# SingleRust/SingleRust

Hardware: AMD Instinct MI355X
Metric: cells/sec end-to-end normalise->HVG->50-PC PCA; SpMM achieved HBM GB/s vs peak (higher is better)
Workload: dtype f32

## Files before the change

### singlerust_amd/csrc/pca_solve.hip

```cpp
#include "pca_internal.hpp"

namespace srx {

#include "spmm.inl"

#include "iterate.inl"

template <typename VT, typename PT>
static int32_t launch_fwd(srx_ctx* ctx, const Tiled& c, const PT* P, const PT* cvec, PT* Y, double* scores = nullptr,
                          int n_pc = 0, int ld = 0) {
    const double out_bytes = scores ? (double)c.n_rows * n_pc * 8.0 : (double)c.n_rows * L * sizeof(PT);
    const double bytes = (double)c.nnz * (4.0 + sizeof(VT)) + (double)((uint64_t)c.nt * c.n_rows + 1) * 8.0 + out_bytes +
                         (double)c.k * L * sizeof(PT);
    const size_t lds = (size_t)KT * L * sizeof(PT);
    constexpr int kRowsPerWg = (kFwdThreads / 16) * FwdCfg<PT>::kRows;
    const uint64_t n_blocks = (c.n_rows + kRowsPerWg - 1) / kRowsPerWg;
    const int per_cu = sizeof(PT) == 4 ? 2 : 1;
    uint64_t grid = (uint64_t)ctx->n_cus * per_cu;
    if (grid > n_blocks) grid = n_blocks;
    if (grid < 1) grid = 1;
    ProfScope ps(ctx, SRX_K_SPMM_FWD, bytes);
    SRX_HIP(ctx, hipFuncSetAttribute((const void*)k_spmm_fwd<VT, PT>, hipFuncAttributeMaxDynamicSharedMemorySize,
                                     (int)lds));
    hipLaunchKernelGGL((k_spmm_fwd<VT, PT>), dim3((unsigned)grid), dim3(kFwdThreads), lds, ctx->stream, c.tptr,
                       (const GramPk<VT>*)c.tpk, c.n_rows, c.nt, c.k, P, cvec, Y, scores, n_pc, ld ? ld : n_pc);
    SRX_HIP(ctx, hipGetLastError());
    return SRX_OK;
}

template <typename PT>
static int fwd_rows_q(int k) {
    const size_t budget = 163840 - 64;
    for (int q = sizeof(PT) == 4 ? 4 : 2; q >= 1; q >>= 1)
        if ((size_t)k * 4 * q * sizeof(PT) <= budget) return q;
    return 0;
}

template <typename VT, typename PT>
static int32_t launch_fwd_rows(srx_ctx* ctx, const RowMajor& r, const PT* P, const PT* cvec, int n_cols, double* scores, PT* Y,
                               int ld) {
    const int Qr = fwd_rows_q<PT>(r.k);
    auto go = [&](auto qtag, auto rtag, auto cltag, int k_lo, int k_hi, int accumulate) -> int32_t {
        constexpr int Q = decltype(qtag)::value;
        constexpr bool RANGE = decltype(rtag)::value;
        constexpr int CL = decltype(cltag)::value;
        constexpr int C = CL * Q;
        const int n_slices = (n_cols + C - 1) / C;
        const int ldp = C;
        const size_t lds = (size_t)(k_hi - k_lo) * ldp * sizeof(PT);
        const uint64_t groups = kFwdRowsThreads / Q;
        uint64_t n_wg = (r.n_rows + groups - 1) / groups;
        uint64_t cap = std::max<uint64_t>(1, (uint64_t)ctx->n_cus * 8 / n_slices);
        if (cap > 8) cap &= ~(uint64_t)7;
        if (n_wg > cap) n_wg = cap;
        if (n_wg < 1) n_wg = 1;
        const double out_bytes = scores ? (double)r.n_rows * n_cols * 8.0 : (double)r.n_rows * L * sizeof(PT);
        ProfScope ps(ctx, SRX_K_SPMM_FWD, (double)r.nnz * sizeof(GramPk<VT>) + (double)(r.n_rows + 1) * 8.0 + out_bytes +
                                              (double)(k_hi - k_lo) * L * sizeof(PT) + (r.perm ? (double)r.n_rows * 4.0 : 0.0));
        SRX_HIP(ctx, hipFuncSetAttribute((const void*)k_spmm_rows<VT, PT, Q, RANGE, CL>, hipFuncAttributeMaxDynamicSharedMemorySize, (int)lds));
        hipLaunchKernelGGL((k_spmm_rows<VT, PT, Q, RANGE, CL>), dim3((unsigned)(n_wg * n_slices)), dim3(kFwdRowsThreads), lds, ctx->stream,
                           r.ptr, (const GramPk<VT>*)r.pk, (const uint32_t*)r.perm, r.n_rows, r.k, P, cvec, n_cols, scores, Y, ld, ldp,
                           k_lo, k_hi, accumulate, 0);
        SRX_HIP(ctx, hipGetLastError());
        return SRX_OK;
    };
    using No = std::false_type;
    using Yes = std::true_type;
    using C4 = std::integral_constant<int, 4>;
    using C5 = std::integral_constant<int, 5>;
    constexpr int Qmax = sizeof(PT) == 4 ? 4 : 2;
    const int wide_slices = (n_cols + 5 * Qmax - 1) / (5 * Qmax), narrow_slices = (n_cols + 4 * Qmax - 1) / (4 * Qmax);
    const bool wide = Qr == Qmax && (size_t)r.k * 5 * Qmax * sizeof(PT) <= (size_t)163840 && wide_slices < narrow_slices &&
                      wide_slices * 5 * Qmax <= L && sizeof(PT) == 8;
    if (wide) return go(std::integral_constant<int, Qmax>{}, No{}, C5{}, 0, r.k, 0);
    if (Qr == 4) {
        if constexpr (sizeof(PT) == 4) return go(std::integral_constant<int, 4>{}, No{}, C4{}, 0, r.k, 0);
        else return SRX_E_ARG;
    }
    if (Qr == 2) return go(std::integral_constant<int, 2>{}, No{}, C4{}, 0, r.k, 0);
    if (Qr == 1) return go(std::integral_constant<int, 1>{}, No{}, C4{}, 0, r.k, 0);
    const int per = (int)((163840 - 64) / (4 * sizeof(PT)));
    for (int k_lo = 0, i = 0; k_lo < r.k; k_lo += per, ++i)
        SRX_TRY(go(std::integral_constant<int, 1>{}, Yes{}, C4{}, k_lo, std::min(r.k, k_lo + per), i > 0 ? 1 : 0));
    return SRX_OK;
}

int32_t build_row_order(srx_ctx* ctx, RowMajor& r) {
    uint32_t* hist;
    SRX_TRY(scratch(ctx, "pca_rm_lenhist", kLenBins * sizeof(uint32_t), (void**)&hist));
    SRX_TRY(scratch(ctx, "pca_rm_perm", (r.n_rows ? r.n_rows : 1) * sizeof(uint32_t), (void**)&r.perm));
    SRX_HIP(ctx, hipMemsetAsync(hist, 0, kLenBins * sizeof(uint32_t), ctx->stream));
    const unsigned g = (unsigned)((r.n_rows + kLenRowsPerWg - 1) / kLenRowsPerWg + (r.n_rows ? 0 : 1));
    hipLaunchKernelGGL(k_len_hist, dim3(g), dim3(256), 0, ctx->stream, r.ptr, r.n_rows, hist);
    hipLaunchKernelGGL(k_len_scan, dim3(1), dim3(kLenBins), 0, ctx->stream, hist);
    hipLaunchKernelGGL(k_len_scatter, dim3(g), dim3(256), 0, ctx->stream, r.ptr, r.n_rows, hist, r.perm);
    SRX_HIP(ctx, hipGetLastError());
    return SRX_OK;
}

template <typename VT, typename YT>
static int32_t launch_t(srx_ctx* ctx, const Tiled& c, const YT* Y, double* T ) {
    uint64_t want = (uint64_t)(2 * ctx->n_cus) / (uint64_t)c.nt;
    if (want < 1) want = 1;
    uint64_t by_rows = (c.n_rows + 255) / 256;
    if (by_rows < 1) by_rows = 1;
    const uint64_t n_rb = want < by_rows ? want : by_rows;
    const uint64_t rpb = (c.n_rows + n_rb - 1) / n_rb > 0 ? (c.n_rows + n_rb - 1) / n_rb : 1;
    double *part, *part_s;
    SRX_TRY(scratch(ctx, "pca_tpart", n_rb * (size_t)c.k * L * sizeof(double), (void**)&part));
    SRX_TRY(scratch(ctx, "pca_tpart_s", n_rb * L * sizeof(double), (void**)&part_s));
    const size_t lds = (size_t)KT * L * sizeof(double);
    const double bytes = (double)c.nnz * (4.0 + sizeof(VT)) + (double)((uint64_t)c.nt * c.n_rows + 1) * 8.0 +
                         (double)c.n_rows * L * sizeof(YT) + (double)c.k * L * 8.0;
    {
        ProfScope ps(ctx, SRX_K_SPMM_T, bytes);
        SRX_HIP(ctx, hipFuncSetAttribute((const void*)k_spmm_t<VT, YT, double>,
                                         hipFuncAttributeMaxDynamicSharedMemorySize, (int)lds));
        hipLaunchKernelGGL((k_spmm_t<VT, YT, double>), dim3((unsigned)(n_rb * c.nt)), dim3(kTThreads), lds, ctx->stream,
                           c.tptr, (const GramPk<VT>*)c.tpk, c.n_rows, c.k, c.nt, rpb, Y, part, part_s);
        uint64_t tot = (uint64_t)c.k * L + L;
        hipLaunchKernelGGL((k_t_reduce<double>), dim3((unsigned)((tot + 255) / 256)), dim3(256), 0, ctx->stream, part,
                           part_s, c.k, n_rb, T);
    }
    SRX_HIP(ctx, hipGetLastError());
    return SRX_OK;
}

static uint64_t mix64(uint64_t x) {
    x += 0x9E3779B97F4A7C15ull;
    x = (x ^ (x >> 30)) * 0xBF58476D1CE4E5B9ull;
    x = (x ^ (x >> 27)) * 0x94D049BB133111EBull;
    return x ^ (x >> 31);
}

struct Work {
    double *W, *Wp, *T, *A1, *A2, *small, *mu, *d, *gpart;
    double *dHG, *dM, *dM2, *dTheta, *dRho, *dColmax, *dSgn, *dDinv, *dXi;
};

static int32_t alloc_work(srx_ctx* ctx, int k, Work& w) {
    const size_t kl = (size_t)k * L;
    SRX_TRY(scratch(ctx, "pca_W", kl * 8, (void**)&w.W));
    SRX_TRY(scratch(ctx, "pca_Wp", kl * 8, (void**)&w.Wp));
    SRX_TRY(scratch(ctx, "pca_T", (kl + L) * 8, (void**)&w.T));
    SRX_TRY(scratch(ctx, "pca_A1", kl * 8, (void**)&w.A1));
    SRX_TRY(scratch(ctx, "pca_A2", kl * 8, (void**)&w.A2));
    SRX_TRY(scratch(ctx, "pca_small", (6 * L * L + 8 * L + 4 * 16 * 16) * 8, (void**)&w.small));
    SRX_TRY(scratch(ctx, "pca_mu", (size_t)k * 8, (void**)&w.mu));
    SRX_TRY(scratch(ctx, "pca_d", (size_t)k * 8, (void**)&w.d));
    SRX_TRY(scratch(ctx, "pca_g2part", (size_t)kGram2Blocks * 2 * L * L * 8, (void**)&w.gpart));
    w.dHG = w.small;
    w.dM = w.small + 2 * L * L;
    w.dM2 = w.small + 3 * L * L;
    w.dTheta = w.small + 4 * L * L;
    w.dRho = w.dTheta + L;
    w.dColmax = w.dRho + L;
    w.dSgn = w.dColmax + L;
    w.dDinv = w.dSgn + L;
    w.dXi = w.small + 6 * L * L + 8 * L;
    return SRX_OK;
}

static int32_t gram2(srx_ctx* ctx, const Work& w, const double* A, const double* B, int k) {
    int nb = (k + 31) / 32;
    if (nb > kGram2Blocks) nb = kGram2Blocks;
    if (nb < 1) nb = 1;
    hipLaunchKernelGGL(k_gram2_part, dim3(nb), dim3(1024), 0, ctx->stream, A, B, k, w.gpart);
    hipLaunchKernelGGL(k_gram2_reduce, dim3((2 * L * L + 255) / 256), dim3(256), 0, ctx->stream, w.gpart, nb, w.dHG);
    SRX_HIP(ctx, hipGetLastError());
    return SRX_OK;
}

template <typename Fn>
static int32_t graphed(srx_ctx* ctx, bool enable, const std::string& key, Fn&& enqueue) {
    if (!enable || ctx->graphs_off) return enqueue();
    auto it = ctx->graphs.find(key);
    if (it == ctx->graphs.end()) {
        if (ctx->graphs.size() >= 32) {
            for (auto& kv : ctx->graphs) (void)hipGraphExecDestroy(kv.second);
            ctx->graphs.clear();
        }
        if (hipStreamBeginCapture(ctx->stream, hipStreamCaptureModeRelaxed) != hipSuccess) {
            (void)hipGetLastError();
            ctx->graphs_off = true;
            return enqueue();
        }
        ctx->capturing = true;
        const int32_t rc = enqueue();
        ctx->capturing = false;
        hipGraph_t g = nullptr;
        const hipError_t e = hipStreamEndCapture(ctx->stream, &g);
        hipGraphExec_t ex = nullptr;
        if (rc == SRX_OK && e == hipSuccess && g && hipGraphInstantiate(&ex, g, nullptr, nullptr, 0) == hipSuccess) {
            (void)hipGraphDestroy(g);
            it = ctx->graphs.emplace(key, ex).first;
        } else {
            if (g) (void)hipGraphDestroy(g);
            (void)hipGetLastError();
            ctx->graphs_off = true;
            return rc != SRX_OK ? rc : enqueue();
        }
    }
    SRX_HIP(ctx, hipGraphLaunch(it->second, ctx->stream));
    return SRX_OK;
}

template <typename Apply>
static int32_t subspace_iterate(srx_ctx* ctx, const Work& w, int k, int l_act, const Resolved& o, Apply&& apply,
                                const void* apply_id, bool graphable, const int* d_status_sel, double& resid, int& iters,
                                bool& converged, bool acc_apply, bool resume = false, bool* bailed_first = nullptr) {
    const size_t kl = (size_t)k * L;
    const bool use_graph = graphable && !getenv("SRX_NO_GRAPH");
    const bool use_cheb = l_act > o.n_pc && !o.robust && !o.direct;
    constexpr int kSlots = srx_ctx::kAsyncSlots, kSlotDoubles = 8;
    if (!ctx->pin_async) {
        SRX_HIP(ctx, hipHostMalloc((void**)&ctx->pin_async, kSlots * kSlotDoubles * sizeof(double), hipHostMallocDefault));
        for (auto& e : ctx->async_ev) SRX_HIP(ctx, hipEventCreateWithFlags(&e, hipEventDisableTiming));
    }
    int* d_status;
    double* d_res;
    constexpr size_t kStatusBytes = 256;
    SRX_TRY(scratch(ctx, "pca_status", kStatusBytes + (size_t)L * L * sizeof(double), (void**)&d_status));
    double* const d_h1 = reinterpret_cast<double*>(reinterpret_cast<char*>(d_status) + kStatusBytes);
    SRX_TRY(scratch(ctx, "pca_res", kSlots * kSlotDoubles * sizeof(double), (void**)&d_res));
    double* d_ritz;
    SRX_TRY(scratch(ctx, "pca_ritzpart", (size_t)kRitzBlocks * 3 * L * sizeof(double), (void**)&d_ritz));
    SRX_HIP(ctx, hipFuncSetAttribute((const void*)k_jacobi_eig2, hipFuncAttributeMaxDynamicSharedMemorySize, (int)sizeof(J2Lds)));
    char key0[320];
    snprintf(key0, sizeof key0, "k%d l%d p%d w%d r%d n%d s%llu t%a|%p %p %p %p %p %p %p %p %p %p", k, l_act, o.power, o.warm,
             (o.robust ? 1 : 0) + (o.direct ? 2 : 0) + (acc_apply ? 4 : 0), o.n_pc,
             (unsigned long long)o.seed, o.tol, apply_id, (void*)w.W, (void*)w.Wp, (void*)w.A1, (void*)w.A2, (void*)w.small,
             (void*)w.gpart, (void*)d_status, (void*)d_status_sel, (void*)w.T);
    const std::string key_base(key0);


    auto gram1 = [&](const double* A, const double* B) -> int32_t {
        int nb = (k + 31) / 32;
        if (nb > kGram1Blocks) nb = kGram1Blocks;
        hipLaunchKernelGGL(k_gram1_part, dim3(nb), dim3(1024), 0, ctx->stream, A, B, k, d_h1);
        SRX_HIP(ctx, hipGetLastError());
        return 1;
    };
    auto orth = [&](const double* src) -> int32_t {
        if (o.robust) {
            SRX_TRY(gram2(ctx, w, src, src, k));
            hipLaunchKernelGGL(k_chol_factor, dim3(1), dim3(1024), 0, ctx->stream, w.dHG + L * L, l_act, w.dM, w.dDinv, d_status, 1);
        } else {
            const int32_t nb = gram1(src, src);
            if (nb < 0) return nb;
            hipLaunchKernelGGL(k_chol_factor_mfma, dim3(1), dim3(1024), 0, ctx->stream, d_h1, l_act, w.dM, w.dDinv, w.dXi, d_status);
        }
        double* const zT = acc_apply ? w.T : nullptr;
        double* const zWp = acc_apply ? w.Wp : nullptr;
        double* const zA1 = acc_apply ? w.A1 : nullptr;
        if (o.robust)
            hipLaunchKernelGGL(k_trsm_rows, dim3((k + 63) / 64), dim3(64), 0, ctx->stream, src, (const double*)w.dM, (const double*)w.dDinv, k, w.W, zWp, zA1, zT);
        else
            hipLaunchKernelGGL(k_trsm_mfma, dim3((k + 16 * kTrsmTiles - 1) / (16 * kTrsmTiles)), dim3(kTrsmTiles * 64), 0, ctx->stream, src,
                               (const double*)w.dM, (const double*)w.dXi, k, w.W, zWp, zA1, zT);
        SRX_HIP(ctx, hipGetLastError());
        if (o.robust) {
            SRX_TRY(gram2(ctx, w, w.W, w.W, k));
            hipLaunchKernelGGL(k_chol_factor, dim3(1), dim3(1024), 0, ctx->stream, w.dHG + L * L, l_act, w.dM, w.dDinv, d_status, 1);
            hipLaunchKernelGGL(k_trsm_rows, dim3((k + 63) / 64), dim3(64), 0, ctx->stream, (const double*)w.W, (const double*)w.dM, (const double*)w.dDinv, k, w.W,
                               (double*)nullptr, (double*)nullptr, (double*)nullptr);
            SRX_HIP(ctx, hipGetLastError());
        }
        return SRX_OK;
    };
    auto apply_n = [&](const double* src, int n, bool after_orth, const double** out) -> int32_t {
        const double* cur = src;
        double* const cand[3] = {w.Wp, w.A1, acc_apply ? w.T : nullptr};
        bool zero[3] = {acc_apply, acc_apply && after_orth, acc_apply};
        for (int t = 0; t < n; ++t) {
            int pick = -1;
            for (int c = 0; c < 3 && pick < 0; ++c)
                if (cand[c] && cand[c] != cur && zero[c]) pick = c;
            for (int c = 0; c < 3 && pick < 0; ++c)
                if (cand[c] && cand[c] != cur) pick = c;
            SRX_TRY(apply(cur, cand[pick], zero[pick]));
            zero[pick] = false;
            cur = cand[pick];
        }
        *out = cur;
        return SRX_OK;
    };
    auto ritz_kernels = [&](int slot, bool loose = false, bool wp_zero = false) -> int32_t {
        SRX_TRY(apply(w.W, w.Wp, wp_zero || acc_apply));
        {
            const int32_t nb = gram1(w.W, w.Wp);
            if (nb < 0) return nb;
            constexpr double loose_tol2 = 1e-6;
            const double exact_tol2 = std::max(1e-30, (o.tol * 1e-4) * (o.tol * 1e-4));
            hipLaunchKernelGGL(k_jacobi_eig2, dim3(1), dim3(kJ2Threads), sizeof(J2Lds), ctx->stream, d_h1, l_act,
                               w.dM2, w.dTheta, d_status, loose ? loose_tol2 : exact_tol2,
                               o.direct ? l_act : std::min(l_act, o.n_pc + 4));
            hipLaunchKernelGGL(k_ritz_post, dim3(kRitzBlocks), dim3(256), 0, ctx->stream, (const double*)w.W, w.Wp,
                               (const double*)w.dM2, (const double*)w.dTheta, k, w.A1, w.A2, d_ritz, acc_apply ? 1 : 0);
            hipLaunchKernelGGL(k_resid_final, dim3(1), dim3(1024), 0, ctx->stream, (const double*)d_ritz, kRitzBlocks,
                               (const double*)w.dTheta, o.n_pc, l_act, d_status, d_status_sel, w.dRho, w.dColmax,
                               d_res + kSlotDoubles * slot);
        }
        SRX_HIP(ctx, hipGetLastError());
        return SRX_OK;
    };
    auto ritz_readback = [&](int slot) -> int32_t {
        SRX_HIP(ctx, hipMemcpyAsync(ctx->pin_async + kSlotDoubles * slot, d_res + kSlotDoubles * slot,
                                    kSlotDoubles * sizeof(double), hipMemcpyDeviceToHost, ctx->stream));
        SRX_HIP(ctx, hipEventRecord(ctx->async_ev[slot], ctx->stream));
        return SRX_OK;
    };
    auto advance = [&]() -> int32_t {
        const double* res;
        SRX_TRY(apply_n(w.A1, o.power - 1, false, &res));
        return orth(res);
    };
    double spread = 1.0;
    auto collect = [&](int slot, double& r, double& ratio) -> int32_t {
        SRX_HIP(ctx, hipEventSynchronize(ctx->async_ev[slot]));
        r = ctx->pin_async[kSlotDoubles * slot];
        const int st = (int)ctx->pin_async[kSlotDoubles * slot + 1];
        ratio = ctx->pin_async[kSlotDoubles * slot + 2];
        spread = ctx->pin_async[kSlotDoubles * slot + 4];
        if ((int)ctx->pin_async[kSlotDoubles * slot + 3] & 1)
            return fail(ctx, SRX_E_NAN, "NaN gene variance: called `Option::unwrap()` on a `None` value (partial_cmp)");
        if (st & kStatChol) return fail(ctx, SRX_E_NOCONV, "pca: block lost rank (Cholesky pivot <= 0)");
        if (st & kStatEig) return fail(ctx, SRX_E_NOCONV, "pca: l x l eigen-solver did not converge");
        if (r != r) return fail(ctx, SRX_E_NOCONV, "pca: NaN in the Ritz residual");
        return SRX_OK;
    };
    auto plain_sweep = [&]() -> int32_t {
        const double* res;
        SRX_TRY(apply_n(w.W, o.power, true, &res));
        return orth(res);
    };

    auto seg_start = [&]() -> int32_t {
        if (o.direct) {
            SRX_HIP(ctx, hipMemsetAsync(d_status, 0, kStatusBytes + (size_t)L * L * sizeof(double), ctx->stream));
            hipLaunchKernelGGL(k_identity_block, dim3((unsigned)((kl + 255) / 256)), dim3(256), 0, ctx->stream, k, w.W);
            SRX_HIP(ctx, hipGetLastError());
            if (acc_apply) SRX_HIP(ctx, hipMemsetAsync(w.Wp, 0, kl * 8, ctx->stream));
            return ritz_kernels(0, false);
        }
        const bool start_orth = o.robust || o.warm < 1;
        hipLaunchKernelGGL(k_init_block, dim3((unsigned)((kl + 255) / 256)), dim3(256), 0, ctx->stream, o.seed, k, l_act,
                           start_orth ? w.Wp : w.W, acc_apply && !start_orth ? w.Wp : (double*)nullptr,
                           acc_apply ? w.A1 : (double*)nullptr, acc_apply ? w.T : (double*)nullptr, reinterpret_cast<uint32_t*>(d_status),
                           (int)((kStatusBytes + (size_t)L * L * sizeof(double)) / 4));
        if (start_orth) {
            SRX_TRY(orth(w.Wp));
            SRX_TRY(orth(w.W));
        }
        for (int sweep = 0; sweep < o.warm; ++sweep) SRX_TRY(plain_sweep());
        return ritz_kernels(0, true);
    };
    const unsigned cheb_grid = (unsigned)((kl + 255) / 256);
    auto cheb_spec = [&]() -> int32_t {
        hipLaunchKernelGGL(k_cheb_first, dim3(cheb_grid), dim3(256), 0, ctx->stream, w.A1, (const double*)w.A2,
                           (const double*)w.dTheta, l_act, kl);
        SRX_HIP(ctx, hipGetLastError());
        return apply(w.A1, w.Wp, acc_apply);
    };
    auto cheb_filter = [&](int d) -> int32_t {
        double *cur = w.A1, *prev = w.A2;
        for (int j = 1; j < d; ++j) {
            if (j > 1) SRX_TRY(apply(cur, w.Wp, true));
            hipLaunchKernelGGL(k_cheb_step, dim3(cheb_grid), dim3(256), 0, ctx->stream, w.Wp,
                               (const double*)cur, prev, (const double*)w.dTheta, l_act, kl);
            double* t = cur;
            cur = prev;
            prev = t;
        }
        hipLaunchKernelGGL(k_cheb_scale, dim3(cheb_grid), dim3(256), 0, ctx->stream, cur, (const double*)w.dTheta, l_act, d, kl);
        SRX_HIP(ctx, hipGetLastError());
        return orth(cur);
    };
    auto cheb_rest = [&](int d, int d2, int slot) -> int32_t {
        SRX_TRY(cheb_filter(d));
        if (d2 > 0) {
            SRX_TRY(apply(w.W, w.Wp, acc_apply));
            hipLaunchKernelGGL(k_cheb_first2, dim3(cheb_grid), dim3(256), 0, ctx->stream, w.Wp, (const double*)w.W, w.A1, w.A2,
                               (const double*)w.dTheta, l_act, kl);
            SRX_HIP(ctx, hipGetLastError());
            SRX_TRY(apply(w.A1, w.Wp, true));
            SRX_TRY(cheb_filter(d2));
        }
        return ritz_kernels(slot, false, true);
    };
    auto seg_next = [&](bool with_advance, int m, int slot) -> int32_t {
        if (with_advance) SRX_TRY(advance());
        for (int sI = 1; sI < m; ++sI) SRX_TRY(plain_sweep());
        return ritz_kernels(slot);
    };

    resid = INFINITY;
    converged = false;
    iters = 0;
    int n_ritz = 0, slot = 0;
    int q_applied = o.warm * o.power + 1;
    double r_last = INFINITY, rate_meas = 0.0;
    int sweeps_since = 0;
    if (bailed_first) *bailed_first = false;
    if (resume) {
        hipLaunchKernelGGL(k_resid_final, dim3(1), dim3(1024), 0, ctx->stream, (const double*)d_ritz, kRitzBlocks,
                           (const double*)w.dTheta, o.n_pc, l_act, d_status, d_status_sel, w.dRho, w.dColmax, d_res + kSlotDoubles * slot);
        SRX_HIP(ctx, hipGetLastError());
    } else {
        SRX_TRY(graphed(ctx, use_graph, key_base + "|start", seg_start));
    }
    SRX_TRY(ritz_readback(slot));
    for (;;) {
        ++iters;
        ++n_ritz;
        const bool first = n_ritz == 1;
        const bool cheb = use_cheb;
        if (cheb && first) {
            if (!resume) SRX_TRY(graphed(ctx, use_graph, key_base + "|cheb0", cheb_spec));
        } else if (first && !o.direct) SRX_TRY(graphed(ctx, use_graph, key_base + "|adv", advance));
        double r, ratio;
        SRX_TRY(collect(slot, r, ratio));
        resid = r;
        if (getenv("SRX_PCA_TRACE")) {
            fprintf(stderr, "[srx pca] sweep %d (ritz step %d): residual %.3e, theta_l/theta_npc %.3e, %d Jacobi sweeps\n", iters + o.warm,
                    n_ritz, r, ratio, (int)ctx->pin_async[kSlotDoubles * slot + 5]);
            int st[64];
            if (d2h(ctx, st, d_status, sizeof st) == SRX_OK) {
                fprintf(stderr, "[srx pca]   Jacobi off / diag per sweep:");
                for (int q = 0; q <= (int)ctx->pin_async[kSlotDoubles * slot + 5] && q < 32; ++q) {
                    float f;
                    memcpy(&f, &st[16 + q], 4);
                    fprintf(stderr, " %.2e", (double)f);
                }
                fprintf(stderr, "\n");
            }
        }
        if (r <= o.tol) {
            converged = true;
            break;
        }
        if (iters >= o.max_iter) break;
        if (first && o.bail_ratio > 0.0 && ratio > o.bail_ratio) {
            if (getenv("SRX_PCA_TRACE")) fprintf(stderr, "[srx pca] flat tail (theta_l / theta_npc = %.3f): leaving the round to the safe plan\n", ratio);
            if (bailed_first) *bailed_first = cheb;
            break;
        }
        if (cheb) {
            const double ta = ratio > 0 && ratio < 1 ? 2.0 / ratio - 1.0 : 1.0;
            int d = 3;
            if (ta > 1.0) d = (int)std::ceil(std::acosh(std::max(4.0 * r / o.tol, 1.0)) / std::acosh(ta) - 1e-9);
            if (d > q_applied) d = q_applied;
            if (d > 12) d = 12;
            {
                const double t1 = 2.0 * (spread > 1.0 ? spread : 1.0) - 1.0;
                const int d_safe = t1 > 1.0 + 1e-9 ? (int)std::floor(32.9 / std::acosh(t1)) : 12;
                if (d > d_safe) d = d_safe;
            }
            if (d < 2) d = 2;
            int d2 = 0;
            if (ta > 1.0) {
                const int d_need = (int)std::ceil(std::acosh(std::max(4.0 * r / o.tol, 1.0)) / std::acosh(ta) - 1e-9);
                if (d_need > d + 1) {
                    const double t1 = 2.0 * (spread > 1.0 ? spread : 1.0) - 1.0;
                    const int d_safe = t1 > 1.0 + 1e-9 ? (int)std::floor(32.9 / std::acosh(t1)) : 12;
                    d2 = std::min(std::min(d_need - d, 12), std::min(d_safe, q_applied + d));
                    if (d2 < 2) d2 = 0;
                }
            }
            q_applied += d + d2;
            iters += (d + d2 + o.power - 1) / o.power;
            slot = (slot + 1) % kSlots;
            char kn[64];
            snprintf(kn, sizeof kn, "|cheb f%d d%d e%d s%d", first ? 1 : 0, d, d2, slot);
            SRX_TRY(graphed(ctx, use_graph, key_base + kn, [&]() -> int32_t {
                if (!first) SRX_TRY(cheb_spec());
                return cheb_rest(d, d2, slot);
            }));
            SRX_TRY(ritz_readback(slot));
            if (getenv("SRX_PCA_TRACE")) {
                if (d2) fprintf(stderr, "[srx pca] Chebyshev filters of degree %d and %d, a CholeskyQR between them (t_a = %.3f)\n", d, d2, ta);
                else fprintf(stderr, "[srx pca] Chebyshev filter of degree %d (t_a = %.3f)\n", d, ta);
            }
            r_last = INFINITY;
            sweeps_since = 0;
            continue;
        }
        if (r_last < INFINITY && sweeps_since > 0 && r < r_last) rate_meas = std::pow(r / r_last, 1.0 / sweeps_since);
        double rate = rate_meas > 0.0 ? rate_meas : std::pow(ratio < 1.0 ? ratio : 1.0, (double)o.power);
        if (!(rate > 1e-8)) rate = 1e-8;
        if (rate > 0.9) rate = 0.9;
        int m = (int)std::ceil(std::log(o.tol / r) / std::log(rate) - 1e-9);
        if (m < 1) m = 1;
        if (m > 6) m = 6;
        if (iters + m > o.max_iter) m = o.max_iter - iters;
        iters += m - 1;
        slot = (slot + 1) % kSlots;
        {
            const bool with_adv = !first;
            char kn[64];
            snprintf(kn, sizeof kn, "|next a%d m%d s%d", with_adv ? 1 : 0, m, slot);
            SRX_TRY(graphed(ctx, use_graph, key_base + kn, [&]() { return seg_next(with_adv, m, slot); }));
        }
        SRX_TRY(ritz_readback(slot));
        r_last = r;
        sweeps_since = m;
    }
    return SRX_OK;
}

constexpr int kPcaPerRound = 48;
constexpr int kPcaPerRoundSafe = 32;
static std::vector<int> plan_rounds(int k , int n_pc, int per) {
    std::vector<int> counts;
    if (k <= L) {
        counts.push_back(n_pc);
        return counts;
    }
    int done = 0;
    while (done < n_pc) {
        const int take = (k - done <= L) ? n_pc - done : std::min(per, n_pc - done);
        counts.push_back(take);
        done += take;
    }
    return counts;
}

__global__ void k_scale_rows(double* __restrict__ M, const double* __restrict__ s) {
    const int e = blockIdx.x * blockDim.x + threadIdx.x;
    if (e < L * L) M[e] *= s[e / L];
}
__global__ void k_sub_inplace(double* __restrict__ a, const double* __restrict__ b, size_t n) {
    const size_t i = (size_t)blockIdx.x * blockDim.x + threadIdx.x;
    if (i < n) a[i] -= b[i];
}
__global__ void k_lock_columns(double* __restrict__ Vl, double* __restrict__ thl, const double* __restrict__ V,
                               const double* __restrict__ theta, int k, int at, int n) {
    const size_t e = (size_t)blockIdx.x * blockDim.x + threadIdx.x;
    if (e >= (size_t)k * n) return;
    const int i = (int)(e / n), c = (int)(e % n);
    Vl[(size_t)i * L + at + c] = V[(size_t)i * L + c];
    if (i == 0) thl[at + c] = theta[c];
}

__global__ void k_deflate(double* __restrict__ C, int k, const double* __restrict__ V, const double* __restrict__ theta, int n) {
    const uint64_t e = (uint64_t)blockIdx.x * blockDim.x + threadIdx.x;
    if (e >= (uint64_t)k * k) return;
    const int i = (int)(e / k), j = (int)(e % k);
    const double* vi = V + (size_t)i * L;
    const double* vj = V + (size_t)j * L;
    double s = 0.0;
    for (int c = 0; c < n; ++c) s += theta[c] * (vi[c] * vj[c]);
    C[e] -= s;
}

int scores_ld(int n_pc) {
    return (n_pc + 15) / 16 * 16;
}
void result_layout(uint64_t n_rows, int k, int n_pc, int dim, size_t& score_bytes, size_t& small_doubles,
                   std::vector<int>* plan_a_out, std::vector<int>* plan_b_out) {
    const size_t kl = (size_t)k * L;
    const std::vector<int> pa = plan_rounds(dim, n_pc, n_pc <= L - 8 ? n_pc : kPcaPerRound);
    const int n_b = (n_pc + kPcaPerRoundSafe - 1) / kPcaPerRoundSafe;
    const std::vector<int> pb = plan_rounds(dim, n_pc, (n_pc + n_b - 1) / n_b);
    const int rounds_cap = (int)std::max(pa.size(), pb.size());
    score_bytes = (n_rows ? n_rows : 1) * (size_t)scores_ld(n_pc) * 8;
    small_doubles = (size_t)rounds_cap * (kl + 2 * L) + 2 * (size_t)k + 2 + ((size_t)k + 1) / 2;
    if (plan_a_out) *plan_a_out = pa;
    if (plan_b_out) *plan_b_out = pb;
}
int32_t ensure_result_capacity(srx_ctx* ctx, srx_pca_state& st, size_t need) {
    if (st.scores_cap < need) {
        if (st.d_scores) SRX_HIP(ctx, hipFree(st.d_scores));
        st.d_scores = nullptr;
        st.scores_cap = 0;
        SRX_HIP(ctx, hipMalloc((void**)&st.d_scores, need));
        st.scores_cap = need;
    }
    return SRX_OK;
}

template <typename VT, typename PT>
int32_t run_pca(srx_ctx* ctx, const RowMajor* parts, int n_parts, const Tiled* t256p, double* gram_packed,
                       const Resolved& o, const SelDev& sel, int l_act, double n_cells, srx_pca_state& st) {
    const RowMajor* rmp = n_parts == 1 ? &parts[0] : nullptr;
    const int k = parts[0].k;
    struct { uint64_t n_rows, max_rows; } cc{0, 0};
    for (int i = 0; i < n_parts; ++i) {
        cc.n_rows += parts[i].n_rows;
        cc.max_rows = std::max(cc.max_rows, parts[i].n_rows);
    }
    const size_t kl = (size_t)k * L;
    Work w;
    st.d_small = nullptr;
    SRX_TRY(alloc_work(ctx, k, w));
    if (o.center) w.mu = sel.d_mu;
    else SRX_HIP(ctx, hipMemsetAsync(w.mu, 0, (size_t)k * 8, ctx->stream));
    w.d = sel.d_dinv;
    PT *P, *cvec, *Y;
    SRX_TRY(scratch(ctx, "pca_P", (kl + L) * sizeof(PT), (void**)&P));
    cvec = P + kl;
    SRX_TRY(scratch(ctx, "pca_Y", (cc.max_rows ? cc.max_rows : 1) * (size_t)L * sizeof(PT), (void**)&Y));

    double resid = INFINITY;
    int iters = 0;
    bool converged = false;
    const int n_pc = o.n_pc;
    const int dim = o.direct ? k : (int)std::min<double>((double)k, n_cells - (o.center ? 1.0 : 0.0));
    std::vector<int> plan_a, plan_b;
    size_t score_bytes, small_doubles;
    result_layout(cc.n_rows, k, n_pc, dim, score_bytes, small_doubles, &plan_a, &plan_b);
    SRX_TRY(ensure_result_capacity(ctx, st, score_bytes + small_doubles * 8));
    double* const d_small = st.d_scores + score_bytes / 8;
    auto finish_round = [&](int r, int col0, int n_r) -> int32_t {
        double* blk = d_small + (size_t)r * (kl + 2 * L);
        hipLaunchKernelGGL((k_make_panel_mb<PT>), dim3(kPanelBlocks), dim3(1024), 0, ctx->stream, (const double*)w.A2, (const double*)w.d,
                           (const double*)w.mu, (const double*)w.dColmax, (const double*)w.dTheta, k, P, w.gpart, w.dSgn, blk);
        hipLaunchKernelGGL((k_cvec_reduce<PT>), dim3(1), dim3(L), 0, ctx->stream, (const double*)w.gpart, kPanelBlocks, o.center, cvec);
        SRX_HIP(ctx, hipGetLastError());
        uint64_t row0 = 0;
        const int ld_s = scores_ld(n_pc);
        if (t256p) {
            SRX_TRY((launch_fwd<VT, PT>(ctx, *t256p, P, cvec, Y, st.d_scores + col0, n_r, ld_s)));
        } else {
            for (int i = 0; i < n_parts; ++i) {
                SRX_TRY((launch_fwd_rows<VT, PT>(ctx, parts[i], P, cvec, n_r, st.d_scores + row0 * (size_t)ld_s + col0, (PT*)nullptr, ld_s)));
                row0 += parts[i].n_rows;
            }
        }
        return SRX_OK;
    };
    const bool acc_apply = o.solver == 1;
    bool bailed_first = false;
    auto run_plan = [&](const std::vector<int>& plan, int budget, bool robust, auto& apply, const void* apply_id, bool graphable,
                        auto& reset, auto& deflate, double bail = 0.0, bool resume = false) -> int32_t {
        if (!resume) SRX_TRY(reset());
        resid = 0.0;
        converged = true;
        iters = 0;
        int done = 0;
        const int rounds = (int)plan.size();
        for (int r = 0; r < rounds; ++r) {
            Resolved o_r = o;
            o_r.n_pc = plan[r];
            o_r.max_iter = budget;
            o_r.seed = o.seed + (uint64_t)r;
            o_r.bail_ratio = bail;
            if (robust) {
                o_r.robust = true;
                o_r.warm = o.warm * o.power;
                o_r.power = 1;
                o_r.max_iter = budget * o.power;
            }
            const int l_r = rounds == 1 ? l_act : std::min(L, dim - done);
            double resid_r = INFINITY;
            int iters_r = 0;
            bool conv_r = false;
            {
                ProfScope ps_it(ctx, SRX_K_ITERATE, (double)k * k * 8.0);
                SRX_TRY(subspace_iterate(ctx, w, k, l_r, o_r, apply, apply_id, graphable, sel.d_status, resid_r,
                                         iters_r, conv_r, acc_apply, resume && r == 0 && l_r == l_act, &bailed_first));
            }
            resid = std::max(resid, resid_r);
            iters += iters_r + o.warm;
            if (!conv_r) {
                converged = false;
                return SRX_OK;
            }
            SRX_TRY(finish_round(r, done, o_r.n_pc));
            if (r + 1 < rounds) SRX_TRY(deflate(done, o_r.n_pc));
            done += o_r.n_pc;
        }
        st.rounds = (uint32_t)rounds;
        st.round_counts = plan;
        return SRX_OK;
    };
    auto solve = [&](auto& apply, const void* apply_id, bool graphable, auto& reset, auto& deflate) -> int32_t {
        const bool have_b = plan_b.size() > plan_a.size();
        if (getenv("SRX_PCA_ROBUST")) {
            SRX_TRY(run_plan(have_b ? plan_b : plan_a, o.max_iter, true, apply, apply_id, graphable, reset, deflate));
            iters -= o.warm;
            return SRX_OK;
        }
        int32_t rc = run_plan(plan_a, have_b && plan_a.size() == 1 ? std::min(o.max_iter, 40) : o.max_iter, false, apply, apply_id,
                              graphable, reset, deflate, have_b && plan_a.size() == 1 ? 0.93 : 0.0);
        if (have_b && (rc == SRX_E_NOCONV || (rc == SRX_OK && !converged))) {
            if (getenv("SRX_PCA_TRACE"))
                fprintf(stderr, "[srx pca] plan A (%zu round(s)) %s at residual %.3e: rounds of <= %d components instead\n",
                        plan_a.size(), rc == SRX_OK ? "stalled" : "broke down", resid, plan_b[0]);
            const int spent = iters;
            const bool resume = rc == SRX_OK && bailed_first && plan_a.size() == 1;
            rc = run_plan(plan_b, o.max_iter, false, apply, apply_id, graphable, reset, deflate, 0.0, resume);
            iters += resume ? 0 : spent;
        }
        if (rc == SRX_E_NOCONV) {
            if (getenv("SRX_PCA_TRACE")) fprintf(stderr, "[srx pca] breakdown again: robust mode (CholeskyQR3 after every application)\n");
            const int spent = iters;
            rc = run_plan(have_b ? plan_b : plan_a, o.max_iter, true, apply, apply_id, graphable, reset, deflate);
            iters += spent;
        }
        SRX_TRY(rc);
        iters -= o.warm;
        return SRX_OK;
    };
    if (o.solver == 1) {
        double* C;
        SRX_TRY(scratch(ctx, "pca_C", (size_t)k * k * 8, (void**)&C));
        double* Pk = gram_packed;
        const size_t n_packed = gram_packed_count(k);
        if (!Pk) {
            Range r_("srx:gram");
            SRX_TRY(scratch(ctx, "pca_gpacked", n_packed * sizeof(double), (void**)&Pk));
            bool reduced = false;
            SRX_TRY(launch_gram<VT>(ctx, *rmp, Pk, &reduced, true));
            if (!reduced) SRX_TRY(allreduce_f64(ctx, Pk, n_packed));
        } else {
            SRX_TRY(allreduce_f64(ctx, Pk, n_packed));
        }
        auto reset = [&]() -> int32_t {
            hipLaunchKernelGGL(k_gram_expand, dim3((unsigned)(((size_t)k * k + 255) / 256)), dim3(256), 0, ctx->stream, Pk,
                               k, (const double*)w.d, (const double*)w.mu, o.center, n_cells, C);
            SRX_HIP(ctx, hipGetLastError());
            return SRX_OK;
        };
        auto apply = [&](const double* Win, double* Wout, bool out_zeroed) -> int32_t {
            ProfScope ps(ctx, SRX_K_DENSE, (double)k * k * 8.0 + 2.0 * k * L * 8.0);
            if (!out_zeroed) SRX_HIP(ctx, hipMemsetAsync(Wout, 0, kl * 8, ctx->stream));
            hipLaunchKernelGGL(k_dense_apply, dim3((k + 31) / 32, kDenseSplit), dim3(kDenseWaves * 64), kDenseLds, ctx->stream, C, Win, k, Wout);
            SRX_HIP(ctx, hipGetLastError());
            return SRX_OK;
        };
        auto deflate = [&](int, int n_r) -> int32_t {
            hipLaunchKernelGGL(k_deflate, dim3((unsigned)(((size_t)k * k + 255) / 256)), dim3(256), 0, ctx->stream, C, k,
                               (const double*)w.A2, (const double*)w.dTheta, n_r);
            SRX_HIP(ctx, hipGetLastError());
            return SRX_OK;
        };
        Range r_("srx:iterate");
        SRX_HIP(ctx, hipFuncSetAttribute((const void*)k_dense_apply, hipFuncAttributeMaxDynamicSharedMemorySize, (int)kDenseLds));
        SRX_TRY(solve(apply, C, true, reset, deflate));
    } else {
        if (n_parts != 1 || !t256p) return fail(ctx, SRX_E_ARG, "pca: the SpMM solver needs the matrix resident in one piece");
        const Tiled& t256 = *t256p;
        double* v_lock;
        SRX_TRY(scratch(ctx, "pca_lock", (kl + L) * 8, (void**)&v_lock));
        double* th_lock = v_lock + kl;
        int n_lock = 0;
        auto reset = [&]() -> int32_t {
            n_lock = 0;
            SRX_HIP(ctx, hipMemsetAsync(v_lock, 0, (kl + L) * 8, ctx->stream));
            return SRX_OK;
        };
        auto apply = [&](const double* Win, double* Wout, bool) -> int32_t {
            hipLaunchKernelGGL((k_make_panel<PT>), dim3(1), dim3(1024), 0, ctx->stream, Win, w.d, w.mu,
                               (const double*)nullptr, k, o.center, P, cvec);
            SRX_HIP(ctx, hipGetLastError());
            if (parts[0].pk && fwd_rows_q<PT>(k) >= 2)
                SRX_TRY((launch_fwd_rows<VT, PT>(ctx, parts[0], P, cvec, L, (double*)nullptr, Y, L)));
            else SRX_TRY((launch_fwd<VT, PT>(ctx, t256, P, cvec, Y)));
            SRX_TRY((launch_t<VT, PT>(ctx, t256, Y, w.T)));
            SRX_TRY(allreduce_f64(ctx, w.T, kl + L));
            hipLaunchKernelGGL(k_finish_t, dim3((unsigned)((kl + 255) / 256)), dim3(256), 0, ctx->stream, w.T, w.d, w.mu,
                               k, o.center, Wout);
            SRX_HIP(ctx, hipGetLastError());
            if (n_lock > 0) {
                SRX_TRY(gram2(ctx, w, v_lock, Win, k));
                hipLaunchKernelGGL(k_scale_rows, dim3((L * L + 255) / 256), dim3(256), 0, ctx->stream, w.dHG, (const double*)th_lock);
                hipLaunchKernelGGL(k_right_mul, dim3(128), dim3(256), 0, ctx->stream, (const double*)v_lock, (const double*)w.dHG, k, w.T);
                hipLaunchKernelGGL(k_sub_inplace, dim3((unsigned)((kl + 255) / 256)), dim3(256), 0, ctx->stream, Wout, (const double*)w.T, kl);
                SRX_HIP(ctx, hipGetLastError());
            }
            return SRX_OK;
        };
        auto deflate = [&](int, int n_r) -> int32_t {
            if (n_lock + n_r > L) return fail(ctx, SRX_E_ARG, "pca: more than %d locked vectors in the matrix-free solver", L);
            hipLaunchKernelGGL(k_lock_columns, dim3((unsigned)(((size_t)k * n_r + 255) / 256)), dim3(256), 0, ctx->stream, v_lock,
                               th_lock, (const double*)w.A2, (const double*)w.dTheta, k, n_lock, n_r);
            SRX_HIP(ctx, hipGetLastError());
            n_lock += n_r;
            return SRX_OK;
        };
        SRX_TRY(solve(apply, nullptr, false, reset, deflate));
    }
    st.d_small = d_small;
    st.info.n_iter = (uint32_t)(iters + o.warm);
    st.info.residual = resid;
    if (!converged)
        return fail(ctx, SRX_E_NOCONV, "pca: subspace iteration stopped at max_iter=%d with residual %.3e > tol %.3e",
                    o.max_iter, resid, o.tol);
    return SRX_OK;
}

int32_t resolve_opts(srx_ctx* ctx, const srx_pca_opts* opts, int k, uint64_t Ng, bool f32, Resolved& o, int& l_act) {
    if (k < 2 || Ng < 5) return fail(ctx, SRX_E_SHAPE, "pca_inplace needs >= 2 selected features and >= 5 cells (k=%d, N=%llu)",
                                     k, (unsigned long long)Ng);
    int want = (!opts || opts->n_components < 0) ? 2 : opts->n_components;
    o.n_pc = std::min(want, k);
    o.center = (!opts || opts->center < 0) ? 1 : (opts->center != 0);
    o.scale = (!opts || opts->scale < 0) ? 1 : (opts->scale != 0);
    o.max_iter = (opts && opts->max_iter > 0) ? opts->max_iter : 0;
    o.tol = (opts && opts->tol > 0) ? opts->tol : 0.0;
    o.seed = opts ? opts->seed : 0;
    o.solver = opts ? opts->solver : 0;
    if (o.solver < 0 || o.solver > 2) return fail(ctx, SRX_E_ARG, "pca: solver must be 0 (auto), 1 (gram) or 2 (spmm)");
    if (o.solver == 0) o.solver = k <= 16384 ? 1 : 2;
    if (o.max_iter == 0) o.max_iter = o.solver == 1 ? 200 : 600;
    o.power = o.solver == 1 ? 3 : 1;
    o.warm = o.solver == 1 ? 2 : 0;
    if (o.solver == 1 && k > 16384) return fail(ctx, SRX_E_ARG, "pca: the Gram solver holds a k x k f64 matrix; k=%d is too large", k);
    if (o.tol == 0.0) o.tol = f32 ? 1e-7 : 1e-9;
    if (o.n_pc < 1) return fail(ctx, SRX_E_ARG, "pca: n_components must be >= 1");
    if (opts && opts->block != 0 && opts->block != L) return fail(ctx, SRX_E_ARG, "pca: only block = %d is built", L);
    const uint64_t rank_bound = std::min<uint64_t>((uint64_t)k, Ng - (o.center ? 1 : 0));
    if ((uint64_t)o.n_pc > rank_bound && !(k <= L && o.solver == 1))
        return fail(ctx, SRX_E_ARG, "pca: n_components %d exceeds the rank of the data (min(k, N%s) = %llu)", o.n_pc,
                    o.center ? " - 1" : "", (unsigned long long)rank_bound);
    l_act = (int)std::min<uint64_t>((uint64_t)L, rank_bound);
    if (k <= L && o.solver == 1) {
        o.direct = true;
        l_act = k;
    }
    if (o.n_pc > l_act && o.solver != 1)
        return fail(ctx, SRX_E_ARG, "pca: n_components %d exceeds what the %d-column block resolves (max %d)", o.n_pc, L, l_act);
    if (rank_bound > (uint64_t)L && o.n_pc > L - 8 && o.solver != 1)
        return fail(ctx, SRX_E_ARG, "pca: n_components %d > %d needs the Gram solver (k <= 16384, opts.solver = 1)", o.n_pc, L - 8);
    return SRX_OK;
}

int32_t stash_results(srx_ctx* ctx, srx_pca_state& st, int k, int n_pc, const SelDev& sel) {
    const size_t kl = (size_t)k * L;
    double* sm = st.d_small + (size_t)st.rounds * (kl + 2 * L);
    CopySegs cs;
    cs.src[0] = (const uint32_t*)sel.d_mu;       cs.dst[0] = (uint32_t*)sm;                          cs.words[0] = (uint32_t)k * 2;
    cs.src[1] = (const uint32_t*)sel.d_sd;       cs.dst[1] = (uint32_t*)(sm + k);                    cs.words[1] = (uint32_t)k * 2;
    cs.src[2] = (const uint32_t*)sel.d_trace;    cs.dst[2] = (uint32_t*)(sm + 2 * (size_t)k);        cs.words[2] = 2;
    cs.src[3] = (const uint32_t*)sel.d_sel_rank; cs.dst[3] = (uint32_t*)(sm + 2 * (size_t)k + 2);    cs.words[3] = (uint32_t)k;
    hipLaunchKernelGGL(k_copy_segs, dim3(16), dim3(256), 0, ctx->stream, cs);
    SRX_HIP(ctx, hipGetLastError());
    st.sel.clear();
    st.k = (uint32_t)k;
    st.n_pc = (uint32_t)n_pc;
    st.host_pending = true;
    st.valid = true;
    return SRX_OK;
}

template int32_t run_pca<float, float>(srx_ctx*, const RowMajor*, int, const Tiled*, double*, const Resolved&, const SelDev&, int, double,
                                        srx_pca_state&);
template int32_t run_pca<float, double>(srx_ctx*, const RowMajor*, int, const Tiled*, double*, const Resolved&, const SelDev&, int, double,
                                         srx_pca_state&);
template int32_t run_pca<double, double>(srx_ctx*, const RowMajor*, int, const Tiled*, double*, const Resolved&, const SelDev&, int, double,
                                          srx_pca_state&);

}

using namespace srx;

extern "C" {

int32_t srx_spmm(srx_mat* m, const uint64_t* sel, uint64_t k64, const double* panel, double* y_out, double* t_out,
                 double* gram_out) {
    if (!m || !sel) return fail(m ? m->ctx : nullptr, SRX_E_ARG, "null argument");
    if ((y_out || t_out) && !panel) return fail(m->ctx, SRX_E_ARG, "srx_spmm: panel is required for y/t");
    if (m->csc) return fail(m->ctx, SRX_E_FORMAT, "srx_spmm walks cells: convert the CSC matrix with srx_matrix_to_csr");
    srx_ctx* ctx = m->ctx;
    SRX_HIP(ctx, hipSetDevice(ctx->device));
    const int k = (int)k64;
    for (int s = 1; s < k; ++s)
        if (sel[s] <= sel[s - 1]) return fail(ctx, SRX_E_ARG, "srx_spmm: sel must be strictly ascending");
    SelDev sd;
    SRX_TRY(select_list(m, sel, k64, 0, 0, sd, false));
    RowMajor crm;
    Tiled c256;
    SRX_TRY(compact_selection(m, sd.d_bits, sd.n_words, k, crm));
    SRX_TRY(retile(m, crm, c256));
    const size_t kl = (size_t)k * L;
    double* T;
    SRX_TRY(scratch(ctx, "pca_T", (kl + L) * 8, (void**)&T));
    auto run = [&](auto vt, auto pt) -> int32_t {
        using VT = decltype(vt);
        using PT = decltype(pt);
        if (y_out || t_out) {
            const Tiled& c = c256;
            PT *P, *Y;
            SRX_TRY(scratch(ctx, "pca_P", (kl + L) * sizeof(PT), (void**)&P));
            SRX_TRY(scratch(ctx, "pca_Y", (c.n_rows ? c.n_rows : 1) * (size_t)L * sizeof(PT), (void**)&Y));
            std::vector<PT> hp(kl + L, PT(0));
            for (size_t e = 0; e < kl; ++e) hp[e] = (PT)panel[e];
            SRX_TRY(h2d(ctx, P, hp.data(), (kl + L) * sizeof(PT)));
            if (getenv("SRX_SPMM_ROWS") && atoi(getenv("SRX_SPMM_ROWS"))) {
                SRX_TRY((launch_fwd_rows<VT, PT>(ctx, crm, P, P + kl, L, (double*)nullptr, Y, L)));
            } else {
                SRX_TRY((launch_fwd<VT, PT>(ctx, c, P, P + kl, Y)));
            }
            if (y_out) {
                std::vector<PT> hy(c.n_rows * (size_t)L);
                SRX_TRY(d2h(ctx, hy.data(), Y, hy.size() * sizeof(PT)));
                for (size_t e = 0; e < hy.size(); ++e) y_out[e] = (double)hy[e];
            }
            if (t_out) {
                SRX_TRY((launch_t<VT, PT>(ctx, c, Y, T)));
                SRX_TRY(d2h(ctx, t_out, T, kl * 8));
            }
        }
        if (gram_out) {
            double *C, *Pk;
            SRX_TRY(scratch(ctx, "pca_C", (size_t)k * k * 8, (void**)&C));
            SRX_TRY(scratch(ctx, "pca_gpacked", gram_packed_count(k) * sizeof(double), (void**)&Pk));
            SRX_HIP(ctx, hipMemsetAsync(Pk, 0, gram_packed_count(k) * sizeof(double), ctx->stream));
            SRX_TRY(launch_gram<VT>(ctx, crm, Pk));
            hipLaunchKernelGGL(k_gram_expand, dim3((unsigned)(((size_t)k * k + 255) / 256)), dim3(256), 0, ctx->stream, Pk,
                               k, (const double*)nullptr, (const double*)nullptr, 0, 0.0, C);
            SRX_HIP(ctx, hipGetLastError());
            SRX_TRY(d2h(ctx, gram_out, C, (size_t)k * k * 8));
        }
        return SRX_OK;
    };
    return is_f32(m) ? run(float{}, float{}) : run(double{}, double{});
}

}
```

Before: 134.2 million.

## Fuse Chebyshev step and Gram epilogues into the dense apply kernel via ticket counters

Adds a DenseTail epilogue to the dense Gram-matrix apply kernel. A global ticket counter in scratch memory lets the last workgroup perform the Chebyshev recurrence update, the final scaling, and the Gram accumulation that feeds the next orthogonalisation or Ritz step. This removes the separate k_cheb_step, k_cheb_scale and gram1 launches and their extra passes over the k×L panels. The first Chebyshev product is now reused from the Ritz post kernel (y1 flag). The change relies on kernel-side code in the includes that is not shown, and it adds grid-wide completion counting that has to be correct under graph replay.

After: 134.7 million, median of 6. About the same (+0.4%).

```diff
diff --git a/singlerust_amd/csrc/pca_solve.hip b/singlerust_amd/csrc/pca_solve.hip
--- a/singlerust_amd/csrc/pca_solve.hip
+++ b/singlerust_amd/csrc/pca_solve.hip
@@ -225,6 +225,15 @@
     SRX_TRY(scratch(ctx, "pca_res", kSlots * kSlotDoubles * sizeof(double), (void**)&d_res));
     double* d_ritz;
     SRX_TRY(scratch(ctx, "pca_ritzpart", (size_t)kRitzBlocks * 3 * L * sizeof(double), (void**)&d_ritz));
+    constexpr int kTickWords = 1024;
+    unsigned* d_tick;
+    const bool tick_new = ctx->scratch.find("pca_tickets") == ctx->scratch.end();
+    SRX_TRY(scratch(ctx, "pca_tickets", kTickWords * sizeof(unsigned), (void**)&d_tick));
+    if (tick_new) SRX_HIP(ctx, hipMemsetAsync(d_tick, 0, kTickWords * sizeof(unsigned), ctx->stream));
+    const bool fuse = acc_apply && !o.robust && (k + 31) / 32 < kTickWords;
+    auto tail = [&](const double* cur, double* prev, int scale_d, const double* gA, bool gram) {
+        return DenseTail{d_tick, cur, prev, (const double*)w.dTheta, l_act, scale_d, gram ? d_h1 : nullptr, gA};
+    };
     SRX_HIP(ctx, hipFuncSetAttribute((const void*)k_jacobi_eig2, hipFuncAttributeMaxDynamicSharedMemorySize, (int)sizeof(J2Lds)));
     char key0[320];
     snprintf(key0, sizeof key0, "k%d l%d p%d w%d r%d n%d s%llu t%a|%p %p %p %p %p %p %p %p %p %p", k, l_act, o.power, o.warm,
@@ -241,13 +250,15 @@
         SRX_HIP(ctx, hipGetLastError());
         return 1;
     };
-    auto orth = [&](const double* src) -> int32_t {
+    auto orth = [&](const double* src, bool gram_done = false) -> int32_t {
         if (o.robust) {
             SRX_TRY(gram2(ctx, w, src, src, k));
             hipLaunchKernelGGL(k_chol_factor, dim3(1), dim3(1024), 0, ctx->stream, w.dHG + L * L, l_act, w.dM, w.dDinv, d_status, 1);
         } else {
-            const int32_t nb = gram1(src, src);
-            if (nb < 0) return nb;
+            if (!gram_done) {
+                const int32_t nb = gram1(src, src);
+                if (nb < 0) return nb;
+            }
             hipLaunchKernelGGL(k_chol_factor_mfma, dim3(1), dim3(1024), 0, ctx->stream, d_h1, l_act, w.dM, w.dDinv, w.dXi, d_status);
         }
         double* const zT = acc_apply ? w.T : nullptr;
@@ -268,7 +279,7 @@
         }
         return SRX_OK;
     };
-    auto apply_n = [&](const double* src, int n, bool after_orth, const double** out) -> int32_t {
+    auto apply_n = [&](const double* src, int n, bool after_orth, const double** out, bool* gram_done = nullptr) -> int32_t {
         const double* cur = src;
         double* const cand[3] = {w.Wp, w.A1, acc_apply ? w.T : nullptr};
         bool zero[3] = {acc_apply, acc_apply && after_orth, acc_apply};
@@ -278,25 +289,39 @@
                 if (cand[c] && cand[c] != cur && zero[c]) pick = c;
             for (int c = 0; c < 3 && pick < 0; ++c)
                 if (cand[c] && cand[c] != cur) pick = c;
-            SRX_TRY(apply(cur, cand[pick], zero[pick]));
+            if (fuse && gram_done && t == n - 1) {
+                const DenseTail tl = tail(nullptr, nullptr, 0, nullptr, true);
+                SRX_TRY(apply(cur, cand[pick], zero[pick], &tl));
+                *gram_done = true;
+            } else {
+                SRX_TRY(apply(cur, cand[pick], zero[pick]));
+            }
             zero[pick] = false;
             cur = cand[pick];
         }
         *out = cur;
         return SRX_OK;
     };
-    auto ritz_kernels = [&](int slot, bool loose = false, bool wp_zero = false) -> int32_t {
-        SRX_TRY(apply(w.W, w.Wp, wp_zero || acc_apply));
+    auto ritz_kernels = [&](int slot, bool loose = false, bool wp_zero = false, bool y1 = false) -> int32_t {
+        if (fuse) {
+            const DenseTail tl = tail(nullptr, nullptr, 0, w.W, true);
+            SRX_TRY(apply(w.W, w.Wp, wp_zero || acc_apply, &tl));
+        } else {
+            SRX_TRY(apply(w.W, w.Wp, wp_zero || acc_apply));
+        }
         {
-            const int32_t nb = gram1(w.W, w.Wp);
-            if (nb < 0) return nb;
+            if (!fuse) {
+                const int32_t nb = gram1(w.W, w.Wp);
+                if (nb < 0) return nb;
+            }
             constexpr double loose_tol2 = 1e-6;
             const double exact_tol2 = std::max(1e-30, (o.tol * 1e-4) * (o.tol * 1e-4));
             hipLaunchKernelGGL(k_jacobi_eig2, dim3(1), dim3(kJ2Threads), sizeof(J2Lds), ctx->stream, d_h1, l_act,
                                w.dM2, w.dTheta, d_status, loose ? loose_tol2 : exact_tol2,
                                o.direct ? l_act : std::min(l_act, o.n_pc + 4));
             hipLaunchKernelGGL(k_ritz_post, dim3(kRitzBlocks), dim3(256), 0, ctx->stream, (const double*)w.W, w.Wp,
-                               (const double*)w.dM2, (const double*)w.dTheta, k, w.A1, w.A2, d_ritz, acc_apply ? 1 : 0);
+                               (const double*)w.dM2, (const double*)w.dTheta, k, w.A1, w.A2, d_ritz, acc_apply ? 1 : 0,
+                               y1 ? 1 : 0, l_act);
             hipLaunchKernelGGL(k_resid_final, dim3(1), dim3(1024), 0, ctx->stream, (const double*)d_ritz, kRitzBlocks,
                                (const double*)w.dTheta, o.n_pc, l_act, d_status, d_status_sel, w.dRho, w.dColmax,
                                d_res + kSlotDoubles * slot);
@@ -312,8 +337,9 @@
     };
     auto advance = [&]() -> int32_t {
         const double* res;
-        SRX_TRY(apply_n(w.A1, o.power - 1, false, &res));
-        return orth(res);
+        bool gram_done = false;
+        SRX_TRY(apply_n(w.A1, o.power - 1, false, &res, &gram_done));
+        return orth(res, gram_done);
     };
     double spread = 1.0;
     auto collect = [&](int slot, double& r, double& ratio) -> int32_t {
@@ -331,8 +357,9 @@
     };
     auto plain_sweep = [&]() -> int32_t {
         const double* res;
-        SRX_TRY(apply_n(w.W, o.power, true, &res));
-        return orth(res);
+        bool gram_done = false;
+        SRX_TRY(apply_n(w.W, o.power, true, &res, &gram_done));
+        return orth(res, gram_done);
     };
 
     auto seg_start = [&]() -> int32_t {
@@ -353,38 +380,47 @@
             SRX_TRY(orth(w.W));
         }
         for (int sweep = 0; sweep < o.warm; ++sweep) SRX_TRY(plain_sweep());
-        return ritz_kernels(0, true);
+        return ritz_kernels(0, true, false, use_cheb);
     };
     const unsigned cheb_grid = (unsigned)((kl + 255) / 256);
     auto cheb_spec = [&]() -> int32_t {
+        return apply(w.A1, w.Wp, acc_apply);
+    };
+    auto cheb_y1 = [&]() -> int32_t {
         hipLaunchKernelGGL(k_cheb_first, dim3(cheb_grid), dim3(256), 0, ctx->stream, w.A1, (const double*)w.A2,
                            (const double*)w.dTheta, l_act, kl);
         SRX_HIP(ctx, hipGetLastError());
-        return apply(w.A1, w.Wp, acc_apply);
-    };
-    auto cheb_filter = [&](int d) -> int32_t {
+        return SRX_OK;
+    };
+    auto cheb_filter = [&](int d, bool z_ready) -> int32_t {
         double *cur = w.A1, *prev = w.A2;
+        bool gram_done = false;
         for (int j = 1; j < d; ++j) {
-            if (j > 1) SRX_TRY(apply(cur, w.Wp, true));
-            hipLaunchKernelGGL(k_cheb_step, dim3(cheb_grid), dim3(256), 0, ctx->stream, w.Wp,
-                               (const double*)cur, prev, (const double*)w.dTheta, l_act, kl);
+            const int scale_d = j == d - 1 ? d : 0;
+            if (fuse && !(j == 1 && z_ready)) {
+                const DenseTail tl = tail(cur, prev, scale_d, nullptr, scale_d > 0);
+                SRX_TRY(apply(cur, w.Wp, true, &tl));
+                gram_done = scale_d > 0;
+            } else {
+                if (!(j == 1 && z_ready)) SRX_TRY(apply(cur, w.Wp, j > 1 || acc_apply));
+                hipLaunchKernelGGL(k_cheb_step, dim3(cheb_grid), dim3(256), 0, ctx->stream, w.Wp,
+                                   (const double*)cur, prev, (const double*)w.dTheta, l_act, scale_d, kl);
+                SRX_HIP(ctx, hipGetLastError());
+            }
             double* t = cur;
             cur = prev;
             prev = t;
         }
-        hipLaunchKernelGGL(k_cheb_scale, dim3(cheb_grid), dim3(256), 0, ctx->stream, cur, (const double*)w.dTheta, l_act, d, kl);
-        SRX_HIP(ctx, hipGetLastError());
-        return orth(cur);
-    };
-    auto cheb_rest = [&](int d, int d2, int slot) -> int32_t {
-        SRX_TRY(cheb_filter(d));
+        return orth(cur, gram_done);
+    };
+    auto cheb_rest = [&](int d, int d2, int slot, bool z_ready) -> int32_t {
+        SRX_TRY(cheb_filter(d, z_ready));
         if (d2 > 0) {
             SRX_TRY(apply(w.W, w.Wp, acc_apply));
             hipLaunchKernelGGL(k_cheb_first2, dim3(cheb_grid), dim3(256), 0, ctx->stream, w.Wp, (const double*)w.W, w.A1, w.A2,
                                (const double*)w.dTheta, l_act, kl);
             SRX_HIP(ctx, hipGetLastError());
-            SRX_TRY(apply(w.A1, w.Wp, true));
-            SRX_TRY(cheb_filter(d2));
+            SRX_TRY(cheb_filter(d2, false));
         }
         return ritz_kernels(slot, false, true);
     };
@@ -473,8 +509,8 @@
             char kn[64];
             snprintf(kn, sizeof kn, "|cheb f%d d%d e%d s%d", first ? 1 : 0, d, d2, slot);
             SRX_TRY(graphed(ctx, use_graph, key_base + kn, [&]() -> int32_t {
-                if (!first) SRX_TRY(cheb_spec());
-                return cheb_rest(d, d2, slot);
+                if (!first) SRX_TRY(cheb_y1());
+                return cheb_rest(d, d2, slot, first);
             }));
             SRX_TRY(ritz_readback(slot));
             if (getenv("SRX_PCA_TRACE")) {
@@ -722,10 +758,11 @@
             SRX_HIP(ctx, hipGetLastError());
             return SRX_OK;
         };
-        auto apply = [&](const double* Win, double* Wout, bool out_zeroed) -> int32_t {
+        auto apply = [&](const double* Win, double* Wout, bool out_zeroed, const DenseTail* tl = nullptr) -> int32_t {
             ProfScope ps(ctx, SRX_K_DENSE, (double)k * k * 8.0 + 2.0 * k * L * 8.0);
             if (!out_zeroed) SRX_HIP(ctx, hipMemsetAsync(Wout, 0, kl * 8, ctx->stream));
-            hipLaunchKernelGGL(k_dense_apply, dim3((k + 31) / 32, kDenseSplit), dim3(kDenseWaves * 64), kDenseLds, ctx->stream, C, Win, k, Wout);
+            hipLaunchKernelGGL(k_dense_apply, dim3((k + 31) / 32, kDenseSplit), dim3(kDenseWaves * 64), kDenseLds, ctx->stream, C, Win, k, Wout,
+                               tl ? *tl : DenseTail{});
             SRX_HIP(ctx, hipGetLastError());
             return SRX_OK;
         };
@@ -750,7 +787,8 @@
             SRX_HIP(ctx, hipMemsetAsync(v_lock, 0, (kl + L) * 8, ctx->stream));
             return SRX_OK;
         };
-        auto apply = [&](const double* Win, double* Wout, bool) -> int32_t {
+        auto apply = [&](const double* Win, double* Wout, bool, const DenseTail* tl = nullptr) -> int32_t {
+            if (tl) return fail(ctx, SRX_E_ARG, "pca: the matrix-free solver has no fused epilogues");
             hipLaunchKernelGGL((k_make_panel<PT>), dim3(1), dim3(1024), 0, ctx->stream, Win, w.d, w.mu,
                                (const double*)nullptr, k, o.center, P, cvec);
             SRX_HIP(ctx, hipGetLastError());
```
